# andrewdalpino/UltraZoom

Hardware: NVIDIA B200
Metric: output_mpx_per_s (higher is better)
Workload: dtype bf16

## Files before the change

### include/mewzoom_b200.h

```cpp
#ifndef MEWZOOM_B200_H_
#define MEWZOOM_B200_H_

#include <stddef.h>
#include <stdint.h>

#ifdef __cplusplus
extern "C" {
#endif

#define MZ_ABI_VERSION 4

typedef enum mz_status {
  MZ_OK = 0,
  MZ_ERR_INVALID = -1,
  MZ_ERR_CUDA = -2,
  MZ_ERR_UNSUPPORTED = -3,
  MZ_ERR_WORKSPACE = -4,
  MZ_ERR_STATE = -5
} mz_status;

#define MZ_FLAG_CLAMP01 1u
#define MZ_FLAG_SIMT_CONV 2u
#define MZ_FLAG_IO_U8 8u
#define MZ_FLAG_U8_TRUNC 16u
// ... 110 lines not shown
int mz_bicubic_f32(const float* x_dev, float* y_dev, int32_t planes, int32_t H, int32_t W, int32_t r,
                   void* stream);

int mz_stem_pack(const float* x_dev, const float* w_dev, const float* bias_dev, float* zf_dev, void* zb_dev,
                 int32_t B, int32_t H, int32_t W, int32_t Cp, int32_t zb_pitch, int32_t operand_dtype, void* stream);

int mz_conv3x3(const void* in_dev, const void* wpacked_dev, int32_t mode, const float* film_dev,
               void* out16_dev, float* zf_dev, int32_t B, int32_t H, int32_t W, int32_t cin_p, int32_t in_pitch,
               int32_t cout_p, int32_t out_pitch, int32_t zf_pitch, int32_t operand_dtype, int32_t use_tc,
               const mz_conv_tune* tune, void* stream);

int mz_head_shuffle_add(const void* zb_dev, const void* wpacked_dev, const float* x_dev, float* y_dev,
                        int32_t B, int32_t H, int32_t W, int32_t cin_p, int32_t in_pitch, int32_t r,
                        int32_t skip_mode, int32_t clamp01, int32_t operand_dtype, int32_t use_tc,
                        const mz_conv_tune* tune, void* stream);

int mz_yuv420_to_rgb16(const void* yuv_dev, uint16_t* rgb_dev, int32_t B, int32_t H, int32_t W, uint32_t flags, void* stream);
int mz_rgb16_to_yuv420(const uint16_t* rgb_dev, void* yuv_dev, int32_t B, int32_t H, int32_t W, uint32_t flags, void* stream);

int mz_pack_conv_weight(const float* w_host, int32_t cout, int32_t cin, int32_t cout_p, int32_t cin_p,
                        int32_t operand_dtype, void* dst_dev, size_t* bytes);

int mz_control_film(const float* c_dev, int32_t c_rows, const float* w_dev ,
                    const float* b_dev , float* film_dev , int32_t L, int32_t B,
                    int32_t F, int32_t hC, int32_t hCp, void* stream);

int mz_put_plane_async(void* dst, size_t dpitch, const void* src, size_t spitch, size_t width_bytes, size_t height,
                       void* stream);

int mz_ipc_frame_create(size_t bytes, void** dev_ptr, void* handle64);
int mz_ipc_frame_open(const void* handle64, void** dev_ptr);
int mz_ipc_frame_close(void* dev_ptr, int32_t owner);

#define MZ_MATH_TF32 0
#define MZ_MATH_FP32 1

int mz_adaptive_mix(const float* x_dev, const float* z_dev, const float* wt_dev, float alpha_logit, float* out_dev,
                    void* out16_dev, int64_t npix, int32_t C, int32_t pitch, int32_t operand_dtype, int32_t math, void* stream);

int mz_pixel_crush(const float* in_dev, const float* wt_dev, float* out_dev, void* out16_dev, int32_t B, int32_t H, int32_t W,
                   int32_t Cin, int32_t Cout, int32_t factor, int32_t pitch_in, int32_t pitch_out, int32_t operand_dtype,
                   int32_t math, void* stream);

int mz_quality_assessor(const float* in_dev, const float* wt_dev, const float* bias_dev, float* out_dev, int32_t B, int32_t H,
                        int32_t W, int32_t C, int32_t F, int32_t pitch_in, void* stream);

int mz_pixel_shuffle_nhwc(const float* in_dev, float* out_dev, void* out16_dev, int32_t B, int32_t H, int32_t W, int32_t C,
                          int32_t r, int32_t pitch_in, int32_t pitch_out, int32_t operand_dtype, void* stream);

int mz_crop_feature_maps(const float* in_dev, float* out_dev, int32_t B, int32_t H, int32_t W, int32_t C, int32_t target_h,
                         int32_t target_w, int32_t pitch_in, int32_t pitch_out, void* stream);

int mz_probe_umma(int32_t kc, int32_t row_shift, int32_t base_offset_mode, float* max_abs_err_out);
int mz_probe_set_gap(int32_t burst_iters, int32_t gap_cycles, int32_t commit_in_gap);
int mz_probe_mma_rate(int32_t n, int32_t kc, int32_t iters, int32_t ctas, int32_t distinct_a,
                      int32_t distinct_d, int32_t a_row_shift, float* cycles_per_mma_out);

int mz_padded_channels(int32_t c);

int mz_zb_pitch(int32_t cp);

#ifdef __cplusplus
}
#endif
#endif
```

### ultrazoom_b200/_native.py

```python
from __future__ import annotations

import ctypes as C
import os
import threading

_HERE = os.path.dirname(os.path.abspath(__file__))
LIB_PATH = os.path.join(_HERE, "lib", "libmewzoom_b200.so")

ABI_VERSION = 4

MZ_OK = 0
MZ_ERR_INVALID = -1
MZ_ERR_CUDA = -2
MZ_ERR_UNSUPPORTED = -3
MZ_ERR_WORKSPACE = -4
MZ_ERR_STATE = -5

FLAG_CLAMP01 = 1
FLAG_SIMT_CONV = 2
FLAG_SKIP_FROM_BUFFER = 4
FLAG_IO_U8 = 8
FLAG_U8_TRUNC = 16
FLAG_X_NHWC = 32
FLAG_Y_NHWC = 64
# ... 43 lines not shown
        ("fuse", C.c_int32),
        ("block", C.c_int32),
        ("seg_rows", C.c_int32),
    ]


_P = C.c_void_p
_I = C.c_int32
SIGNATURES = {
    "mz_last_error": (C.c_char_p, []),
    "mz_abi_version": (C.c_int, []),
    "mz_device_count": (C.c_int, []),
    "mz_model_create": (C.c_int, [C.POINTER(MzConfig), C.POINTER(_P)]),
    "mz_model_destroy": (None, [_P]),
    "mz_model_set_weight": (C.c_int, [_P, _I, _I, _P, C.c_size_t]),
    "mz_model_set_weight_dev": (C.c_int, [_P, _I, _I, _P, C.c_size_t, _P]),
    "mz_model_saturated": (C.c_int, [_P, _I, C.POINTER(_I)]),
    "mz_model_set_tune": (C.c_int, [_P, _I, C.POINTER(MzConvTune)]),
    "mz_model_enable_timing": (C.c_int, [_P, _I]),
    "mz_model_conv_stack_ms": (C.c_int, [_P, C.POINTER(C.c_float)]),
    "mz_workspace_bytes": (C.c_int, [_P, _I, _I, _I, C.POINTER(C.c_size_t)]),
    "mz_workspace_bytes_flags": (C.c_int, [_P, _I, _I, _I, C.c_uint32, C.POINTER(C.c_size_t)]),
    "mz_model_fused_block": (C.c_int, [_P]),
    "mz_block_fused": (C.c_int, [_P, _P, _P, _P, _P, _P, _I, _I, _I, _I, _I, _I, _P]),
    "mz_upscale": (C.c_int, [_P, _P, _P, _I, _P, _I, _I, _I, _P, C.c_size_t, C.c_uint32, _P]),
    "mz_upscale_window": (C.c_int, [_P, _P, _P, _I, _P, C.c_int64, C.c_int64, _I, _I, _I, _I, _I, _I, _I, _P, C.c_size_t,
                                    C.c_uint32, _P]),
    "mz_upscale_stage": (C.c_int, [_P, _P, _P, _I, _P, C.c_int64, C.c_int64, _I, _I, _I, _I, _I, _I, _I, _P, C.c_size_t,
                                   C.c_uint32, _P, _I, _I]),
    "mz_workspace_layout": (C.c_int, [_P, _I, _I, _I, C.POINTER(C.c_size_t), C.POINTER(C.c_size_t), C.POINTER(C.c_size_t),
                                      C.POINTER(_I), C.POINTER(_I)]),
    "mz_enable_peer_access": (C.c_int, [_I, _I]),
    "mz_ipc_frame_create": (C.c_int, [C.c_size_t, C.POINTER(C.c_void_p), _P]),
    "mz_ipc_frame_open": (C.c_int, [_P, C.POINTER(C.c_void_p)]),
    "mz_ipc_frame_close": (C.c_int, [_P, _I]),
    "mz_upscale_host": (C.c_int, [_P, _P, _P, _I, _P, _I, _I, _I, C.c_uint32]),
    "mz_upscale_host_async": (C.c_int, [_P, _I, _P, _P, _I, _P, _I, _I, _I, C.c_uint32]),
    "mz_upscale_host_wait": (C.c_int, [_P, _I]),
    "mz_put_plane_async": (C.c_int, [_P, C.c_size_t, _P, C.c_size_t, C.c_size_t, C.c_size_t, _P]),
    "mz_bicubic_f32": (C.c_int, [_P, _P, _I, _I, _I, _I, _P]),
    "mz_stem_pack": (C.c_int, [_P, _P, _P, _P, _P, _I, _I, _I, _I, _I, _I, _P]),
    "mz_conv3x3": (C.c_int, [_P, _P, _I, _P, _P, _P, _I, _I, _I, _I, _I, _I, _I, _I, _I, _I, C.POINTER(MzConvTune), _P]),
    "mz_head_shuffle_add": (C.c_int, [_P, _P, _P, _P, _I, _I, _I, _I, _I, _I, _I, _I, _I, _I, C.POINTER(MzConvTune), _P]),
    "mz_yuv420_to_rgb16": (C.c_int, [_P, _P, _I, _I, _I, C.c_uint32, _P]),
    "mz_rgb16_to_yuv420": (C.c_int, [_P, _P, _I, _I, _I, C.c_uint32, _P]),
    "mz_pack_conv_weight": (C.c_int, [_P, _I, _I, _I, _I, _I, _P, C.POINTER(C.c_size_t)]),
    "mz_control_film": (C.c_int, [_P, _I, _P, _P, _P, _I, _I, _I, _I, _I, _P]),
    "mz_adaptive_mix": (C.c_int, [_P, _P, _P, C.c_float, _P, _P, C.c_int64, _I, _I, _I, _I, _P]),
    "mz_pixel_crush": (C.c_int, [_P, _P, _P, _P, _I, _I, _I, _I, _I, _I, _I, _I, _I, _I, _P]),
    "mz_quality_assessor": (C.c_int, [_P, _P, _P, _P, _I, _I, _I, _I, _I, _I, _P]),
    "mz_pixel_shuffle_nhwc": (C.c_int, [_P, _P, _P, _I, _I, _I, _I, _I, _I, _I, _I, _P]),
    "mz_crop_feature_maps": (C.c_int, [_P, _P, _I, _I, _I, _I, _I, _I, _I, _I, _P]),
    "mz_probe_umma": (C.c_int, [_I, _I, _I, C.POINTER(C.c_float)]),
    "mz_probe_set_gap": (C.c_int, [_I, _I, _I]),
    "mz_probe_mma_rate": (C.c_int, [_I, _I, _I, _I, _I, _I, _I, C.POINTER(C.c_float)]),
    "mz_padded_channels": (C.c_int, [_I]),
    "mz_zb_pitch": (C.c_int, [_I]),
}

_lib = None
_lock = threading.Lock()


def load(build_if_missing: bool = True) -> C.CDLL:
    global _lib
    with _lock:
        if _lib is not None:
            return _lib
        if build_if_missing:
            from . import build as _build

            try:
                _build.build_locked()
            except RuntimeError:
                if not os.path.exists(LIB_PATH):
                    raise
        if not os.path.exists(LIB_PATH):
            raise RuntimeError(f"{LIB_PATH} is missing; run `python -m ultrazoom_b200.build`")
        try:
            lib = C.CDLL(LIB_PATH)
        except OSError as e:
            raise RuntimeError(f"cannot load {LIB_PATH}: {e}") from e
        for name, (res, args) in SIGNATURES.items():
            fn = getattr(lib, name)
            fn.restype = res
            fn.argtypes = args
        if lib.mz_abi_version() != ABI_VERSION:
            raise RuntimeError(f"ABI mismatch: library reports {lib.mz_abi_version()}, binding expects {ABI_VERSION}")
        _lib = lib
        return lib


def last_error() -> str:
    return load().mz_last_error().decode("utf-8", "replace")


def check(rc: int) -> None:
    if rc == MZ_OK:
        return
    msg = last_error()
    if rc == MZ_ERR_INVALID:
        raise AssertionError(msg)
    raise RuntimeError(f"mewzoom_b200 error {rc}: {msg}")


def dtype_code(dt) -> int:
# ... 14 lines not shown
```

### ultrazoom_b200/csrc/block_fused.cu

```cuda
#include <stdlib.h>

#include "kernels.cuh"

namespace mz {

namespace fb {
constexpr int kC = 48, kHC = 96;
constexpr int kStrip = 126;
constexpr int kThreads = 384;
constexpr int kZbStages = 4, kHidBufs = 2, kAcc1Stages = 2, kNB = 4, kRingBlocks = kNB + 2;
constexpr uint32_t kW1Tile = 48 * 32;
constexpr uint32_t kW1Bytes = 27 * kW1Tile;
constexpr uint32_t kW2Tile = 72 * 64;
constexpr uint32_t kW2Bytes = 9 * kW2Tile;
constexpr uint32_t kZbSub = 4352;
constexpr uint32_t kZbRow = 3 * kZbSub, kZbRowTx = 3 * 130 * 32;
constexpr uint32_t kHidChunk = 128 * 64, kHidBuf = 3 * kHidChunk;
constexpr uint32_t kStageZ = 3 * 32 * 64, kStageO = 3 * 32 * 32, kStageWarp = kStageZ + kStageO;

constexpr uint32_t oW1 = 0;
constexpr uint32_t oW2 = oW1 + kW1Bytes;
constexpr uint32_t oZb = oW2 + kW2Bytes;
constexpr uint32_t oHid = oZb + kZbStages * kZbRow;
constexpr uint32_t oStage = (oHid + kHidBufs * kHidBuf + 256 + 1023) & ~1023u;
// ... 171 lines not shown
          }
          if (leader) umma2_commit_mcast(bar_acc2_full + 8 * (pos % kNB), 3);
          __syncwarp();
        }
      }
      for (int i = 0; i <= steps; ++i) {
        if (i < steps) {
          for (int k = (i == 0 ? 0 : 2); k < 3; ++k) {
            const uint32_t c = zcnt + i + k;
            FB_TIMED(0, mbar_wait(bar_zb_full + 8 * (c % kZbStages), (c / kZbStages) & 1u));
          }
          const uint32_t st1 = a1 % kAcc1Stages;
          FB_TIMED(1, mbar_wait(bar_acc1_empty + 8 * st1, ((a1 / kAcc1Stages) & 1u) ^ 1u));
          tc_fence_after();
          const uint32_t d1 = tmem_base + kAcc1Col + st1 * kHC;
          if (leader) {
            if (!(p.dbg & 4))
#pragma unroll
            for (int dy = 0; dy < 3; ++dy) {
              const uint32_t arow = base + oZb + ((zcnt + i + dy) % kZbStages) * kZbRow;
#pragma unroll
              for (int dx = 0; dx < 3; ++dx) {
#pragma unroll
                for (int sub = 0; sub < 3; ++sub) {
                  const uint64_t ad = (static_cast<uint64_t>(hi32) << 32) | lo(arow + sub * kZbSub + dx * 32);
                  const uint64_t bd = (static_cast<uint64_t>(hi32) << 32) | lo(base + oW1 + ((dy * 3 + sub) * 3 + dx) * kW1Tile);
                  if (dy == 0 && dx == 0 && sub == 0)
                    umma2_bf16(d1, ad, bd, p.idesc1, 0u);
                  else
                    umma2_acc(d1, ad, bd, p.idesc1);
                }
              }
            }
            umma2_commit_mcast(bar_acc1_full + 8 * st1, 3);
            umma2_commit_mcast(bar_zb_empty + 8 * ((zcnt + i) % kZbStages), 3);
            if (i == steps - 1) {
              umma2_commit_mcast(bar_zb_empty + 8 * ((zcnt + i + 1) % kZbStages), 3);
              umma2_commit_mcast(bar_zb_empty + 8 * ((zcnt + i + 2) % kZbStages), 3);
            }
          }
          __syncwarp();
          ++a1;
        }
        if (i >= 1) {
          const int j = i - 1;
          const uint32_t hb = hcnt % kHidBufs;
          FB_TIMED(2, mbar_wait(bar_hid_full + 8 * hb, (hcnt / kHidBufs) & 1u));
          while (opened <= pos + j + 2) {
            FB_TIMED(3, mbar_wait(bar_acc2_empty + 8 * (opened % kNB), ((opened / kNB) & 1u) ^ 1u));
            ++opened;
          }
          tc_fence_after();
          const uint32_t d2 = tmem_base + kRingCol + ((pos + j) % kNB) * kC;
          if (leader) {
            if (!(p.dbg & 8))
#pragma unroll
            for (int dx = 0; dx < 3; ++dx) {
#pragma unroll
              for (int c = 0; c < 3; ++c) {
#pragma unroll
                for (int ks = 0; ks < 2; ++ks) {
                  const uint64_t ad = (static_cast<uint64_t>(hi64) << 32) | lo(base + oHid + hb * kHidBuf + c * kHidChunk + dx * 64 + ks * 32);
                  const uint64_t bd = (static_cast<uint64_t>(hi64) << 32) | lo(base + oW2 + (dx * 3 + c) * kW2Tile + ks * 32);
                  umma2_acc(d2, ad, bd, p.idesc2);
                }
              }
            }
            umma2_commit_mcast(bar_hid_empty + 8 * hb, 3);
            umma2_commit_mcast(bar_acc2_full + 8 * ((pos + j) % kNB), 3);
            if (j == steps - 1) {
              umma2_commit_mcast(bar_acc2_full + 8 * ((pos + j + 1) % kNB), 3);
              umma2_commit_mcast(bar_acc2_full + 8 * ((pos + j + 2) % kNB), 3);
            }
          }
          __syncwarp();
          ++hcnt;
        }
      }
      zcnt += rows_per_unit;
      pos += rows_per_unit;
    }
  } else if (warp >= 4 && warp < 8) {
    griddep_wait();
    const int q = warp & 3;
    float* film_s = reinterpret_cast<float*>(gen_base + oFilm);
    int film_b = -1;
    float amax = 0.f;
    uint32_t a1 = 0;
    const uint32_t px_row = q * 32 + lane;
    for (int unit = cluster_id; unit < p.n_units; unit += n_clusters) {
      int b, y0, x0;
      unit_geom(unit, b, y0, x0);
      if (b != film_b) {
        named_bar_sync(1, 128);
        for (int i = threadIdx.x - 128; i < 2 * kHC; i += 128) {
          float v = i < kHC ? 1.f : 0.f;
          if (p.film != nullptr) v = __ldg(p.film + static_cast<size_t>(b) * 2 * kHC + i);
          film_s[i] = 0.5f * v;
        }
        named_bar_sync(1, 128);
        film_b = b;
      }
      const int hx = x0 - 1 + static_cast<int>(px_row);
      const bool px_ok = hx >= 0 && hx < p.W;
      for (int i = 0; i < steps; ++i, ++a1) {
        const uint32_t st1 = a1 % kAcc1Stages, hb = a1 % kHidBufs;
        const int hy = y0 - 1 + i;
        const bool keep = px_ok && hy >= 0 && hy < p.H;
        FB_TIMED(0, mbar_wait(bar_acc1_full + 8 * st1, (a1 / kAcc1Stages) & 1u));
        FB_TIMED(1, mbar_wait(bar_hid_empty + 8 * hb, ((a1 / kHidBufs) & 1u) ^ 1u));
        __syncwarp();
        tc_fence_after();
        const uint32_t taddr = tmem_base + (static_cast<uint32_t>(q * 32) << 16) + kAcc1Col + st1 * kHC;
        const uint32_t hrow = base + oHid + hb * kHidBuf + px_row * 64;
#pragma unroll
        for (int c = 0; c < 3; ++c) {
          uint32_t v[32];
          FB_TIMED(2, { tmem_ld32(taddr + c * 32, v); tmem_ld_wait(); });
          const long long t_math = prof_on ? clock64() : 0;
          const float4* sc = reinterpret_cast<const float4*>(film_s + c * 32);
          const float4* sh = reinterpret_cast<const float4*>(film_s + kHC + c * 32);
          uint32_t o[16];
#pragma unroll
          for (int kk = 0; kk < 8; ++kk) {
            const float4 g = sc[kk], h = sh[kk];
            float a0 = silu_h(fmaf(__uint_as_float(v[4 * kk + 0]), g.x, h.x));
            float a1v = silu_h(fmaf(__uint_as_float(v[4 * kk + 1]), g.y, h.y));
            float a2 = silu_h(fmaf(__uint_as_float(v[4 * kk + 2]), g.z, h.z));
            float a3 = silu_h(fmaf(__uint_as_float(v[4 * kk + 3]), g.w, h.w));
            if (!keep) a0 = a1v = a2 = a3 = 0.f;
            if (p.dbg & 2) a0 = a1v = a2 = a3 = __uint_as_float(v[4 * kk]);
            amax = fmaxf(fmaxf(amax, fmaxf(fabsf(a0), fabsf(a1v))), fmaxf(fabsf(a2), fabsf(a3)));
            o[2 * kk] = pack_op2(p.bf16, a0, a1v);
            o[2 * kk + 1] = pack_op2(p.bf16, a2, a3);
          }
          const uint32_t crow = hrow + c * kHidChunk;
#pragma unroll
          for (int ch = 0; ch < 4; ++ch)
            sts128(crow + swz_chunk(px_row, ch, 64) * 16, o[4 * ch], o[4 * ch + 1], o[4 * ch + 2], o[4 * ch + 3]);
          if (prof_on) tick[3] += clock64() - t_math;
        }
        FB_TIMED(4, {
          tc_fence_before();
          fence_proxy_async_smem();
          __syncwarp();
        });
        FB_TIMED(5, {
          if (lane == 0) {
            mbar_arrive_remote(mapa_u32(bar_acc1_empty + 8 * st1, 0));
            mbar_arrive_remote(mapa_u32(bar_hid_full + 8 * hb, 0));
          }
        });
      }
    }
    if (!p.bf16 && p.sat != nullptr && !(amax <= MZ_F16_MAX)) *p.sat = 1u;
  } else if (warp >= 8) {
    griddep_wait();
    const int q = warp & 3;
    const uint32_t st_z = base + oStage + q * kStageWarp, st_o = st_z + kStageZ;
    const uint32_t my_res = bar_res + 8 * (q * 3);
    const CUtensorMap* tmZ = &p.tmZ[q == 3 ? 1 : 0];
    const CUtensorMap* tmO = &p.tmO[q == 3 ? 1 : 0];
    const uint32_t slice_bytes = (q == 3 ? 30u : 32u) * 16 * 4;
    float amax = 0.f;
    const bool lane_live = !(q == 3 && lane >= 30);
    uint32_t pos = 0, rpar = 0;
    bool preloaded = false;
    bool pending_last = false;
    for (int unit = cluster_id; unit < p.n_units; unit += n_clusters) {
      int b, y0, x0;
      unit_geom(unit, b, y0, x0);
      const int xw = x0 + q * 32;
      const int lead = static_cast<int>((static_cast<uint32_t>(y0 + 2) - pos) & 3u);
      for (int rho = -lead; rho < rows_per_unit; ++rho, ++pos) {
        const int y = y0 - 2 + rho;
        const bool store = rho >= 2 && rho < T + 2 && y < p.H && xw < p.W && !(p.dbg & 1);
        const uint32_t k = pos % kNB, par = (pos / kNB) & 1u;
        if (store && lane == 0) {
          if (!preloaded) {
            FB_TIMED(2, bulk_wait_read<0>());
            for (int j = 0; j < 3; ++j) {
              mbar_expect_tx(my_res + 8 * j, slice_bytes);
              tma_load_4d(st_z + j * 2048, tmZ, my_res + 8 * j, j * 16, xw, y, b);
            }
          } else if (pending_last) {
            FB_TIMED(2, bulk_wait_read<0>());
            mbar_expect_tx(my_res + 16, slice_bytes);
            tma_load_4d(st_z + 2 * 2048, tmZ, my_res + 16, 32, xw, y, b);
          }
        }
        FB_TIMED(0, mbar_wait(bar_acc2_full + 8 * k, par));
        __syncwarp();
        tc_fence_after();
        const long long t_body = prof_on ? clock64() : 0;
        const uint32_t lane_base = tmem_base + (static_cast<uint32_t>(q * 32) << 16) + kRingCol;
// ... 263 lines not shown
```

### ultrazoom_b200/csrc/common.cuh

```cuda
#pragma once

#include <cuda.h>
#include <cuda_bf16.h>
#include <cuda_fp16.h>
#include <cuda_runtime.h>
#include <stdint.h>
#include <stdio.h>

#include "../../include/mewzoom_b200.h"

namespace mz {

void set_error(const char* fmt, ...);
int cuda_fail(cudaError_t e, const char* what, const char* file, int line);

#define MZ_CUDA(expr)                                                        \
  do {                                                                       \
    cudaError_t _e = (expr);                                                 \
    if (_e != cudaSuccess) return ::mz::cuda_fail(_e, #expr, __FILE__, __LINE__); \
  } while (0)

#define MZ_REQUIRE(cond, ...)          \
  do {                                 \
    if (!(cond)) {                     \
// ... 170 lines not shown
__device__ __forceinline__ void mbar_arrive_cluster(uint32_t cluster_addr) {
  asm volatile("mbarrier.arrive.release.cluster.shared::cluster.b64 _, [%0];" ::"r"(cluster_addr) : "memory");
}
__device__ __forceinline__ void mbar_arrive_remote(uint32_t cluster_addr) {
  asm volatile("mbarrier.arrive.shared::cluster.b64 _, [%0];" ::"r"(cluster_addr) : "memory");
}
__device__ __forceinline__ void tma2_load_4d(uint32_t dst, const CUtensorMap* m, uint32_t bar_cluster, int c0, int c1,
                                             int c2, int c3) {
  asm volatile(
      "cp.async.bulk.tensor.4d.cta_group::2.shared::cluster.global.mbarrier::complete_tx::bytes [%0], [%1, {%3, %4, %5, "
      "%6}], [%2];" ::"r"(dst),
      "l"(reinterpret_cast<uint64_t>(m)), "r"(bar_cluster), "r"(c0), "r"(c1), "r"(c2), "r"(c3)
      : "memory");
}
__device__ __forceinline__ void tma2_load_3d(uint32_t dst, const CUtensorMap* m, uint32_t bar_cluster, int c0, int c1,
                                             int c2) {
  asm volatile(
      "cp.async.bulk.tensor.3d.cta_group::2.shared::cluster.global.mbarrier::complete_tx::bytes [%0], [%1, {%3, %4, "
      "%5}], [%2];" ::"r"(dst),
      "l"(reinterpret_cast<uint64_t>(m)), "r"(bar_cluster), "r"(c0), "r"(c1), "r"(c2)
      : "memory");
}
__device__ __forceinline__ void tmem_alloc2(uint32_t smem_dst, uint32_t ncols) {
  asm volatile("tcgen05.alloc.cta_group::2.sync.aligned.shared::cta.b32 [%0], %1;" ::"r"(smem_dst), "r"(ncols)
               : "memory");
}
__device__ __forceinline__ void tmem_relinquish2() {
  asm volatile("tcgen05.relinquish_alloc_permit.cta_group::2.sync.aligned;" ::: "memory");
}
__device__ __forceinline__ void tmem_dealloc2(uint32_t taddr, uint32_t ncols) {
  asm volatile("tcgen05.dealloc.cta_group::2.sync.aligned.b32 %0, %1;" ::"r"(taddr), "r"(ncols) : "memory");
}
__device__ __forceinline__ void umma2_bf16(uint32_t d_tmem, uint64_t a_desc, uint64_t b_desc, uint32_t idesc,
                                           uint32_t accumulate) {
  asm volatile(
      "{\n\t"
      ".reg .pred p;\n\t"
      "setp.ne.b32 p, %4, 0;\n\t"
      "tcgen05.mma.cta_group::2.kind::f16 [%0], %1, %2, %3, p;\n\t"
      "}\n" ::"r"(d_tmem),
      "l"(a_desc), "l"(b_desc), "r"(idesc), "r"(accumulate)
      : "memory");
}
__device__ __forceinline__ void umma2_acc(uint32_t d_tmem, uint64_t a_desc, uint64_t b_desc, uint32_t idesc) {
  asm volatile(
      "{\n\t"
      ".reg .pred p;\n\t"
      "setp.eq.u32 p, 0, 0;\n\t"
      "tcgen05.mma.cta_group::2.kind::f16 [%0], %1, %2, %3, p;\n\t"
      "}\n" ::"r"(d_tmem),
      "l"(a_desc), "l"(b_desc), "r"(idesc)
      : "memory");
}
__device__ __forceinline__ void umma2_commit_mcast(uint32_t bar, uint16_t cta_mask) {
  asm volatile(
      "tcgen05.commit.cta_group::2.mbarrier::arrive::one.shared::cluster.multicast::cluster.b64 [%0], %1;" ::"r"(bar),
      "h"(cta_mask)
      : "memory");
}

__device__ __forceinline__ void griddep_launch_dependents() { asm volatile("griddepcontrol.launch_dependents;" ::: "memory"); }
__device__ __forceinline__ void griddep_wait() { asm volatile("griddepcontrol.wait;" ::: "memory"); }

__device__ __forceinline__ void tmem_alloc(uint32_t smem_dst, uint32_t ncols) {
  asm volatile("tcgen05.alloc.cta_group::1.sync.aligned.shared::cta.b32 [%0], %1;" ::"r"(smem_dst), "r"(ncols)
               : "memory");
}
__device__ __forceinline__ void tmem_relinquish() {
  asm volatile("tcgen05.relinquish_alloc_permit.cta_group::1.sync.aligned;" ::: "memory");
}
__device__ __forceinline__ void tmem_dealloc(uint32_t taddr, uint32_t ncols) {
  asm volatile("tcgen05.dealloc.cta_group::1.sync.aligned.b32 %0, %1;" ::"r"(taddr), "r"(ncols) : "memory");
}
__device__ __forceinline__ void tc_fence_before() {
  asm volatile("tcgen05.fence::before_thread_sync;" ::: "memory");
}
__device__ __forceinline__ void tc_fence_after() {
  asm volatile("tcgen05.fence::after_thread_sync;" ::: "memory");
}
__device__ __forceinline__ void umma_bf16(uint32_t d_tmem, uint64_t a_desc, uint64_t b_desc, uint32_t idesc,
                                          uint32_t accumulate) {
  asm volatile(
      "{\n\t"
      ".reg .pred p;\n\t"
      "setp.ne.b32 p, %4, 0;\n\t"
      "tcgen05.mma.cta_group::1.kind::f16 [%0], %1, %2, %3, p;\n\t"
      "}\n" ::"r"(d_tmem),
      "l"(a_desc), "l"(b_desc), "r"(idesc), "r"(accumulate)
      : "memory");
}
__device__ __forceinline__ void umma_acc(uint32_t d_tmem, uint64_t a_desc, uint64_t b_desc, uint32_t idesc) {
  asm volatile(
      "{\n\t"
      ".reg .pred p;\n\t"
      "setp.eq.u32 p, 0, 0;\n\t"
      "tcgen05.mma.cta_group::1.kind::f16 [%0], %1, %2, %3, p;\n\t"
      "}\n" ::"r"(d_tmem),
      "l"(a_desc), "l"(b_desc), "r"(idesc)
      : "memory");
}
__device__ __forceinline__ void umma_commit(uint32_t bar) {
  asm volatile("tcgen05.commit.cta_group::1.mbarrier::arrive::one.shared::cluster.b64 [%0];" ::"r"(bar)
               : "memory");
}
__device__ __forceinline__ void umma_commit_mcast(uint32_t bar, uint16_t cta_mask) {
  asm volatile(
      "tcgen05.commit.cta_group::1.mbarrier::arrive::one.shared::cluster.multicast::cluster.b64 [%0], %1;" ::"r"(bar),
      "h"(cta_mask)
      : "memory");
}
__device__ __forceinline__ void tmem_ld16(uint32_t taddr, uint32_t (&v)[16]) {
  asm volatile(
      "tcgen05.ld.sync.aligned.32x32b.x16.b32 "
      "{%0, %1, %2, %3, %4, %5, %6, %7, %8, %9, %10, %11, %12, %13, %14, %15}, [%16];"
      : "=r"(v[0]), "=r"(v[1]), "=r"(v[2]), "=r"(v[3]), "=r"(v[4]), "=r"(v[5]), "=r"(v[6]), "=r"(v[7]),
        "=r"(v[8]), "=r"(v[9]), "=r"(v[10]), "=r"(v[11]), "=r"(v[12]), "=r"(v[13]), "=r"(v[14]), "=r"(v[15])
      : "r"(taddr)
      : "memory");
}
__device__ __forceinline__ void tmem_ld32(uint32_t taddr, uint32_t (&v)[32]) {
  asm volatile(
      "tcgen05.ld.sync.aligned.32x32b.x32.b32 "
      "{%0, %1, %2, %3, %4, %5, %6, %7, %8, %9, %10, %11, %12, %13, %14, %15, "
      "%16, %17, %18, %19, %20, %21, %22, %23, %24, %25, %26, %27, %28, %29, %30, %31}, [%32];"
      : "=r"(v[0]), "=r"(v[1]), "=r"(v[2]), "=r"(v[3]), "=r"(v[4]), "=r"(v[5]), "=r"(v[6]), "=r"(v[7]),
        "=r"(v[8]), "=r"(v[9]), "=r"(v[10]), "=r"(v[11]), "=r"(v[12]), "=r"(v[13]), "=r"(v[14]), "=r"(v[15]),
        "=r"(v[16]), "=r"(v[17]), "=r"(v[18]), "=r"(v[19]), "=r"(v[20]), "=r"(v[21]), "=r"(v[22]), "=r"(v[23]),
        "=r"(v[24]), "=r"(v[25]), "=r"(v[26]), "=r"(v[27]), "=r"(v[28]), "=r"(v[29]), "=r"(v[30]), "=r"(v[31])
      : "r"(taddr)
      : "memory");
}
__device__ __forceinline__ void tmem_ld_wait() {
  asm volatile("tcgen05.wait::ld.sync.aligned;" ::: "memory");
}
__device__ __forceinline__ void tmem_zero16(uint32_t taddr) {
  const uint32_t z = 0u;
  asm volatile(
      "tcgen05.st.sync.aligned.32x32b.x16.b32 [%0], "
      "{%1, %1, %1, %1, %1, %1, %1, %1, %1, %1, %1, %1, %1, %1, %1, %1};" ::"r"(taddr),
      "r"(z)
      : "memory");
}
__device__ __forceinline__ void tmem_st_wait() {
  asm volatile("tcgen05.wait::st.sync.aligned;" ::: "memory");
}

__host__ __device__ constexpr uint32_t umma_layout_type(int kc) { return kc == 64 ? 2u : (kc == 32 ? 4u : 6u); }

__device__ __forceinline__ uint64_t umma_smem_desc(uint32_t saddr, uint32_t sbo_bytes, uint32_t layout_type,
                                                   uint32_t base_offset = 0) {
  uint64_t d = 0;
  d |= static_cast<uint64_t>((saddr & 0x3FFFFu) >> 4);
  d |= static_cast<uint64_t>(1) << 16;
  d |= static_cast<uint64_t>((sbo_bytes >> 4) & 0x3FFFu) << 32;
  d |= static_cast<uint64_t>(1) << 46;
  d |= static_cast<uint64_t>(base_offset & 7u) << 49;
  d |= static_cast<uint64_t>(layout_type & 7u) << 61;
  return d;
}
__host__ __device__ constexpr uint32_t umma_idesc_bf16(int m, int n) {
  return (1u << 4) | (1u << 7) | (1u << 10) | (static_cast<uint32_t>(n >> 3) << 17) |
         (static_cast<uint32_t>(m >> 4) << 24);
}
__host__ __device__ constexpr uint32_t umma_idesc_f16(int m, int n) {
  return (1u << 4) | (static_cast<uint32_t>(n >> 3) << 17) | (static_cast<uint32_t>(m >> 4) << 24);
}

__device__ __forceinline__ uint32_t pack_bf16x2(float lo, float hi) {
  __nv_bfloat162 v = __floats2bfloat162_rn(lo, hi);
  return *reinterpret_cast<uint32_t*>(&v);
}
__device__ __forceinline__ uint32_t pack_f16x2(float lo, float hi) {
  uint32_t r;
  asm("cvt.rn.satfinite.f16x2.f32 %0, %1, %2;" : "=r"(r) : "f"(hi), "f"(lo));
  return r;
}
__device__ __forceinline__ uint32_t pack_f16x2_rn(float lo, float hi) {
  uint32_t r;
  asm("cvt.rn.f16x2.f32 %0, %1, %2;" : "=r"(r) : "f"(hi), "f"(lo));
  return r;
}
__device__ __forceinline__ uint32_t pack_op2(int bf16, float lo, float hi) {
  return bf16 ? pack_bf16x2(lo, hi) : pack_f16x2(lo, hi);
}
__device__ __forceinline__ uint32_t pack_shadow2(int bf16, float lo, float hi) {
  return bf16 ? pack_bf16x2(lo, hi) : pack_f16x2_rn(lo, hi);
}
__device__ __forceinline__ float2 unpack_op2(int bf16, uint32_t u) {
  if (bf16) return make_float2(__uint_as_float(u << 16), __uint_as_float(u & 0xffff0000u));
  return __half22float2(*reinterpret_cast<const __half2*>(&u));
}
__device__ __forceinline__ float op_to_float(int bf16, uint16_t v) {
  return bf16 ? __uint_as_float(static_cast<uint32_t>(v) << 16) : __half2float(__ushort_as_half(v));
// ... 22 lines not shown
```

### ultrazoom_b200/csrc/probe.cu

```cuda
#include <vector>

#include "kernels.cuh"

namespace mz {

constexpr int kProbeRows = 384;
constexpr int kProbeN = 64;

struct ProbeParams {
  CUtensorMap tmA, tmB;
  float* out;
  int kc, row_shift, bo_mode;
};

__global__ void __launch_bounds__(128, 1) probe_umma_kernel(const __grid_constant__ ProbeParams p) {
  extern __shared__ uint8_t smem_raw[];
  const uint32_t raw = smem_u32(smem_raw);
  const uint32_t base = (raw + 1023u) & ~1023u;
  uint8_t* gen = smem_raw + (base - raw);
  const int row_bytes = p.kc * 2;
  const uint32_t a_smem = base;
  const uint32_t b_smem = base + kProbeRows * 128;
  const uint32_t bar_full = b_smem + kProbeN * 128;
  const uint32_t bar_done = bar_full + 8;
  const uint32_t tmem_slot = bar_done + 32;
  volatile uint32_t* tmem_gen = reinterpret_cast<volatile uint32_t*>(gen + (tmem_slot - base));
  const int warp = threadIdx.x >> 5, lane = threadIdx.x & 31;

  if (threadIdx.x == 0) {
    mbar_init(bar_full, 1);
    mbar_init(bar_done, 1);
    fence_mbar_init();
  }
  if (warp == 0) {
    tmem_alloc(tmem_slot, 64);
    tmem_relinquish();
  }
  tc_fence_before();
  __syncthreads();
  tc_fence_after();
  const uint32_t tmem_base = *tmem_gen;

  if (threadIdx.x == 0) {
    mbar_expect_tx(bar_full, (kProbeRows + kProbeN) * row_bytes);
    tma_load_2d(a_smem, &p.tmA, bar_full, 0, 0);
    tma_load_2d(a_smem + 192 * row_bytes, &p.tmA, bar_full, 0, 192);
    tma_load_2d(b_smem, &p.tmB, bar_full, 0, 0);
    mbar_wait(bar_full, 0);
    tc_fence_after();
    const uint32_t lt = umma_layout_type(p.kc);
    const uint32_t sbo = 8u * row_bytes;
    const uint32_t idesc = umma_idesc_bf16(128, kProbeN);
    for (int ks = 0; ks < p.kc / 16; ++ks) {
      const uint32_t a_addr = a_smem + p.row_shift * row_bytes + ks * 32;
      const uint32_t bo = p.bo_mode ? ((a_addr >> 7) & 7u) : 0u;
      umma_bf16(tmem_base, umma_smem_desc(a_addr, sbo, lt, bo), umma_smem_desc(b_smem + ks * 32, sbo, lt, 0), idesc,
                ks != 0);
    }
    umma_commit(bar_done);
  }
  mbar_wait(bar_done, 0);
  __syncwarp();
  tc_fence_after();
  const uint32_t taddr = tmem_base + (static_cast<uint32_t>(warp * 32) << 16);
  for (int n0 = 0; n0 < kProbeN; n0 += 16) {
    uint32_t v[16];
    tmem_ld16(taddr + n0, v);
    tmem_ld_wait();
#pragma unroll
    for (int i = 0; i < 16; ++i) p.out[(warp * 32 + lane) * kProbeN + n0 + i] = __uint_as_float(v[i]);
  }
  tc_fence_before();
  __syncthreads();
  if (warp == 0) {
    tc_fence_after();
    tmem_dealloc(tmem_base, 64);
  }
}

struct RateParams {
  float* out;
  int n, kc, iters, distinct_a, distinct_d, a_row_shift;
  int gap_cycles, commit_in_gap;
  int burst_iters;
  uint32_t tmem_cols;
};

__global__ void __launch_bounds__(128, 1) probe_rate_kernel(const RateParams p) {
  extern __shared__ uint8_t smem_raw[];
  const uint32_t raw = smem_u32(smem_raw);
  const uint32_t base = (raw + 1023u) & ~1023u;
  uint8_t* gen = smem_raw + (base - raw);
  const uint32_t a_smem = base;
  const uint32_t b_smem = base + 8 * 16384;
  const uint32_t bar_done = b_smem + 32768;
  const uint32_t tmem_slot = bar_done + 32;
  volatile uint32_t* tmem_gen = reinterpret_cast<volatile uint32_t*>(gen + (tmem_slot - base));
  const int warp = threadIdx.x >> 5;
  for (uint32_t i = threadIdx.x; i < (8 * 16384 + 32768) / 4; i += blockDim.x)
    reinterpret_cast<uint32_t*>(gen)[i] = 0x3c003c00u;
  fence_proxy_async_smem();
  if (threadIdx.x == 0) {
    mbar_init(bar_done, 1);
    mbar_init(bar_done + 16, 1);
    fence_mbar_init();
  }
  if (warp == 0) {
    tmem_alloc(tmem_slot, p.tmem_cols);
    tmem_relinquish();
  }
  tc_fence_before();
  __syncthreads();
  tc_fence_after();
  const uint32_t tmem_base = *tmem_gen;
  if (warp == 1) {
    const int row_bytes = p.kc * 2;
    const uint32_t lt = umma_layout_type(p.kc);
    const uint32_t sbo = 8u * row_bytes;
    const uint32_t idesc = umma_idesc_bf16(128, p.n);
    const uint32_t hi = static_cast<uint32_t>(umma_smem_desc(0, sbo, lt, 0) >> 32);
    const uint32_t lo0 = static_cast<uint32_t>(umma_smem_desc(0, sbo, lt, 0));
    const uint32_t b_lo = lo0 + (b_smem >> 4);
    const uint32_t a_lo = lo0 + ((a_smem + static_cast<uint32_t>(p.a_row_shift * row_bytes)) >> 4);
    const uint32_t a_step = p.distinct_a > 1 ? (16384u >> 4) : 0u;
    const uint32_t d_step = p.distinct_d > 1 ? static_cast<uint32_t>(p.n) : 0u;
    const bool leader = elect_one();
    const uint32_t dynmask = (p.iters & 1) ? 0xffffffffu : static_cast<uint32_t>(p.a_row_shift >> 8);
    const long long t0 = clock64();
    int until_gap = p.burst_iters;
// ... 52 lines not shown
    hB[i] = __float2bfloat16_rn(fB[i]);
  }
  __nv_bfloat16 *dA = nullptr, *dB = nullptr;
  float* dOut = nullptr;
  MZ_CUDA(cudaMalloc(&dA, hA.size() * 2));
  MZ_CUDA(cudaMalloc(&dB, hB.size() * 2));
  MZ_CUDA(cudaMalloc(&dOut, sizeof(float) * 128 * kProbeN));
  MZ_CUDA(cudaMemcpy(dA, hA.data(), hA.size() * 2, cudaMemcpyHostToDevice));
  MZ_CUDA(cudaMemcpy(dB, hB.data(), hB.size() * 2, cudaMemcpyHostToDevice));
  MZ_CUDA(cudaMemset(dOut, 0xff, sizeof(float) * 128 * kProbeN));
  ProbeParams p;
  memset(&p, 0, sizeof(p));
  p.out = dOut;
  p.kc = kc;
  p.row_shift = row_shift;
  p.bo_mode = base_offset_mode;
  const CUtensorMapSwizzle swz =
      kc == 64 ? CU_TENSOR_MAP_SWIZZLE_128B : (kc == 32 ? CU_TENSOR_MAP_SWIZZLE_64B : CU_TENSOR_MAP_SWIZZLE_32B);
  int rc;
  {
    const uint64_t dims[2] = {static_cast<uint64_t>(kc), kProbeRows};
    const uint64_t strides[1] = {static_cast<uint64_t>(kc) * 2};
    const uint32_t box[2] = {static_cast<uint32_t>(kc), 192};
    rc = encode_tmap(&p.tmA, CU_TENSOR_MAP_DATA_TYPE_BFLOAT16, 2, dA, dims, strides, box, swz);
  }
  if (rc == MZ_OK) {
    const uint64_t dims[2] = {static_cast<uint64_t>(kc), kProbeN};
    const uint64_t strides[1] = {static_cast<uint64_t>(kc) * 2};
    const uint32_t box[2] = {static_cast<uint32_t>(kc), kProbeN};
    rc = encode_tmap(&p.tmB, CU_TENSOR_MAP_DATA_TYPE_BFLOAT16, 2, dB, dims, strides, box, swz);
  }
  if (rc == MZ_OK) {
    const int smem = 1024 + kProbeRows * 128 + kProbeN * 128 + 64;
    cudaError_t e = cudaFuncSetAttribute(probe_umma_kernel, cudaFuncAttributeMaxDynamicSharedMemorySize, smem);
    if (e == cudaSuccess) {
      probe_umma_kernel<<<1, 128, smem>>>(p);
      e = cudaGetLastError();
    }
    if (e == cudaSuccess) e = cudaDeviceSynchronize();
    if (e != cudaSuccess) rc = cuda_fail(e, "probe_umma_kernel", __FILE__, __LINE__);
  }
  if (rc == MZ_OK) {
    std::vector<float> out(128 * kProbeN);
    cudaMemcpy(out.data(), dOut, out.size() * sizeof(float), cudaMemcpyDeviceToHost);
    float worst = 0.f;
    for (int m = 0; m < 128; ++m)
      for (int n = 0; n < kProbeN; ++n) {
        float ref = 0.f;
        for (int k = 0; k < kc; ++k) ref += fA[static_cast<size_t>(row_shift + m) * kc + k] * fB[static_cast<size_t>(n) * kc + k];
        float d = fabsf(out[m * kProbeN + n] - ref);
        if (!(d == d)) d = 1e30f;
        if (d > worst) worst = d;
      }
    *max_abs_err_out = worst;
  }
  cudaFree(dA);
  cudaFree(dB);
  cudaFree(dOut);
  return rc;
}

static int g_gap_cycles = 0, g_commit_in_gap = 0, g_burst_iters = 0;
int mz_probe_set_gap(int32_t burst_iters, int32_t gap_cycles, int32_t commit_in_gap) {
  g_burst_iters = burst_iters;
  g_gap_cycles = gap_cycles;
  g_commit_in_gap = commit_in_gap;
  return MZ_OK;
}

int mz_probe_mma_rate(int32_t n, int32_t kc, int32_t iters, int32_t ctas, int32_t distinct_a, int32_t distinct_d,
                      int32_t a_row_shift, float* cycles_per_mma_out) {
  MZ_REQUIRE(a_row_shift >= 0 && a_row_shift <= 64, "probe: a_row_shift must be in [0, 64]");
  MZ_REQUIRE(n >= 16 && n <= 256 && n % 16 == 0, "probe: n must be a multiple of 16 in [16, 256]");
  MZ_REQUIRE(kc == 16 || kc == 32 || kc == 64, "probe: kc must be 16, 32 or 64");
  MZ_REQUIRE(iters > 0 && iters <= (1 << 20) && ctas > 0 && ctas <= 4096, "probe: bad iters/ctas");
  MZ_REQUIRE(distinct_a == 1 || distinct_a == 2 || distinct_a == 4 || distinct_a == 8, "probe: distinct_a must be 1, 2, 4 or 8");
  MZ_REQUIRE(distinct_d >= 1 && distinct_d * n <= 512, "probe: distinct_d * n must fit 512 TMEM columns");
  MZ_REQUIRE(cycles_per_mma_out, "probe: null output");
  float* dOut = nullptr;
  MZ_CUDA(cudaMalloc(&dOut, sizeof(float) * ctas));
  RateParams p;
  p.out = dOut;
  p.n = n;
  p.kc = kc;
  p.iters = iters;
  p.distinct_a = distinct_a;
  p.distinct_d = distinct_d;
  p.a_row_shift = a_row_shift;
  p.gap_cycles = g_gap_cycles;
  p.commit_in_gap = g_commit_in_gap;
  p.burst_iters = g_burst_iters;
  p.tmem_cols = 32;
  while (p.tmem_cols < static_cast<uint32_t>(n * distinct_d)) p.tmem_cols <<= 1;
  const int smem = 1024 + 8 * 16384 + 32768 + 128;
  int rc = MZ_OK;
  cudaError_t e = cudaFuncSetAttribute(probe_rate_kernel, cudaFuncAttributeMaxDynamicSharedMemorySize, smem);
  if (e == cudaSuccess) {
    probe_rate_kernel<<<ctas, 128, smem>>>(p);
    e = cudaGetLastError();
  }
  if (e == cudaSuccess) e = cudaDeviceSynchronize();
  if (e != cudaSuccess) rc = cuda_fail(e, "probe_rate_kernel", __FILE__, __LINE__);
  if (rc == MZ_OK) {
    std::vector<float> out(ctas);
    cudaMemcpy(out.data(), dOut, sizeof(float) * ctas, cudaMemcpyDeviceToHost);
    double sum = 0;
// ... 9 lines not shown
```

### ultrazoom_b200/ops.py

```python
from __future__ import annotations

import ctypes as C
from typing import Optional

import torch
from torch import Tensor

from . import _native


def _stream(t: Tensor) -> int:
    return torch.cuda.current_stream(t.device).cuda_stream


def _need_cuda(*ts: Tensor) -> None:
    for t in ts:
        if t is not None and not t.is_cuda:
            raise RuntimeError("ultrazoom_b200.ops: CUDA tensors required (no CPU fallback)")


def padded_channels(c: int) -> int:
    return _native.load().mz_padded_channels(c)


# ... 117 lines not shown
            inp.data_ptr(), wpacked.data_ptr(), mode, film.data_ptr() if film is not None else None,
            out.data_ptr() + 2 * channel_offset, zf.data_ptr() + 4 * channel_offset if zf is not None else None, B, H, W, cin_p,
            in_pitch if in_pitch != cin_p else 0, cout_p, out_pitch if out_pitch != cout_p else 0,
            zf_pitch if zf_pitch != cout_p else 0, _native.dtype_code(inp.dtype), 1 if use_tc else 0,
            C.byref(tune) if tune is not None else None, _stream(inp)))
    return out


def block_fused(zb: Tensor, w1_packed: Tensor, w2_packed: Tensor, film: Optional[Tensor], zf: Tensor, seg_rows: int = 0,
                max_ctas: int = 0) -> Tensor:
    _need_cuda(zb, w1_packed, w2_packed, zf)
    assert zb.dtype in (torch.float16, torch.bfloat16) and w1_packed.dtype == zb.dtype and w2_packed.dtype == zb.dtype
    zb = zb.contiguous()
    B, H, W, Cc = zb.shape
    assert Cc == 48 and tuple(w1_packed.shape) == (9, 96, 48) and tuple(w2_packed.shape) == (9, 48, 96), "48 / 96 channels only"
    assert zf.is_contiguous() and tuple(zf.shape) == (B, H, W, 48) and zf.dtype == torch.float32
    out = torch.empty_like(zb)
    with torch.cuda.device(zb.device):
        _native.check(_native.load().mz_block_fused(
            zb.data_ptr(), out.data_ptr(), zf.data_ptr(), w1_packed.data_ptr(), w2_packed.data_ptr(),
            film.data_ptr() if film is not None else None, B, H, W, _native.dtype_code(zb.dtype), seg_rows, max_ctas,
            _stream(zb)))
    return out


def head_shuffle_add(zb: Tensor, wpacked: Tensor, r: int, x: Optional[Tensor] = None, y: Optional[Tensor] = None,
                     skip_mode: int = 2, clamp01: bool = False, use_tc: bool = True,
                     tune: Optional[_native.MzConvTune] = None) -> Tensor:
    _need_cuda(zb, wpacked)
    assert zb.dtype in (torch.float16, torch.bfloat16) and wpacked.dtype == zb.dtype
    zb = zb.contiguous()
    B, H, W, in_pitch = zb.shape
    cin_p = wpacked.shape[2]
    assert in_pitch >= cin_p, "weight / activation channel mismatch"
    if y is None:
        assert skip_mode != 1, "skip_mode 1 needs y preloaded with the bicubic image"
        y = torch.empty((B, 3, H * r, W * r), dtype=torch.float32, device=zb.device)
    if x is not None:
        x = x.to(torch.float32).contiguous()
    with torch.cuda.device(zb.device):
        _native.check(_native.load().mz_head_shuffle_add(
            zb.data_ptr(), wpacked.data_ptr(), x.data_ptr() if x is not None else None, y.data_ptr(), B, H, W, cin_p,
            in_pitch if in_pitch != cin_p else 0, r, skip_mode, 1 if clamp01 else 0, _native.dtype_code(zb.dtype), 1 if use_tc else 0, C.byref(tune) if tune is not None else None,
            _stream(zb)))
    return y


def probe_umma(kc: int, row_shift: int, base_offset_mode: int) -> float:
    err = C.c_float()
    _native.check(_native.load().mz_probe_umma(kc, row_shift, base_offset_mode, C.byref(err)))
    return err.value


def probe_mma_rate(n: int, kc: int, iters: int = 2000, ctas: int = 1, distinct_a: int = 1,
                   distinct_d: int = 1, a_row_shift: int = 0) -> float:
    cyc = C.c_float()
    _native.check(_native.load().mz_probe_mma_rate(n, kc, iters, ctas, distinct_a, distinct_d, a_row_shift,
                                                   C.byref(cyc)))
    return cyc.value
```

Baseline: 1108.

## Feed center-tap A operand of fused block second conv from TMEM

In the fused block kernel, the epilogue now also writes the activated hidden tile into TMEM alongside the swizzled shared-memory copy. For the dx==0 taps, the second conv's MMA reads its A operand from TMEM instead of a shared-memory descriptor, which is meant to cut shared-memory read bandwidth pressure on the tensor core. A probe kernel is added to check that TMEM-sourced A produces the same results as SMEM A. The cost is extra tcgen05.st traffic and a store wait in the epilogue. It also risks correctness, since the TMEM A layout and the ring-slot lifetime may not match what the MMA expects.

```diff
diff --git a/include/mewzoom_b200.h b/include/mewzoom_b200.h
--- a/include/mewzoom_b200.h
+++ b/include/mewzoom_b200.h
@@ -186,6 +186,7 @@
                          int32_t target_w, int32_t pitch_in, int32_t pitch_out, void* stream);
 
 int mz_probe_umma(int32_t kc, int32_t row_shift, int32_t base_offset_mode, float* max_abs_err_out);
+int mz_probe_umma_tmem_a(int32_t n, int32_t bf16, int32_t a_col, int32_t* mismatches_out, float* max_abs_err_out);
 int mz_probe_set_gap(int32_t burst_iters, int32_t gap_cycles, int32_t commit_in_gap);
 int mz_probe_mma_rate(int32_t n, int32_t kc, int32_t iters, int32_t ctas, int32_t distinct_a,
                       int32_t distinct_d, int32_t a_row_shift, float* cycles_per_mma_out);
diff --git a/ultrazoom_b200/_native.py b/ultrazoom_b200/_native.py
--- a/ultrazoom_b200/_native.py
+++ b/ultrazoom_b200/_native.py
@@ -119,6 +119,7 @@
     "mz_pixel_shuffle_nhwc": (C.c_int, [_P, _P, _P, _I, _I, _I, _I, _I, _I, _I, _I, _P]),
     "mz_crop_feature_maps": (C.c_int, [_P, _P, _I, _I, _I, _I, _I, _I, _I, _I, _P]),
     "mz_probe_umma": (C.c_int, [_I, _I, _I, C.POINTER(C.c_float)]),
+    "mz_probe_umma_tmem_a": (C.c_int, [_I, _I, _I, C.POINTER(C.c_int32), C.POINTER(C.c_float)]),
     "mz_probe_set_gap": (C.c_int, [_I, _I, _I]),
     "mz_probe_mma_rate": (C.c_int, [_I, _I, _I, _I, _I, _I, _I, C.POINTER(C.c_float)]),
     "mz_padded_channels": (C.c_int, [_I]),
diff --git a/ultrazoom_b200/csrc/block_fused.cu b/ultrazoom_b200/csrc/block_fused.cu
--- a/ultrazoom_b200/csrc/block_fused.cu
+++ b/ultrazoom_b200/csrc/block_fused.cu
@@ -247,6 +247,7 @@
           }
           tc_fence_after();
           const uint32_t d2 = tmem_base + kRingCol + ((pos + j) % kNB) * kC;
+          const uint32_t hid_t = tmem_base + kAcc1Col + (hcnt % kAcc1Stages) * kHC;
           if (leader) {
             if (!(p.dbg & 8))
 #pragma unroll
@@ -255,9 +256,13 @@
               for (int c = 0; c < 3; ++c) {
 #pragma unroll
                 for (int ks = 0; ks < 2; ++ks) {
-                  const uint64_t ad = (static_cast<uint64_t>(hi64) << 32) | lo(base + oHid + hb * kHidBuf + c * kHidChunk + dx * 64 + ks * 32);
                   const uint64_t bd = (static_cast<uint64_t>(hi64) << 32) | lo(base + oW2 + (dx * 3 + c) * kW2Tile + ks * 32);
-                  umma2_acc(d2, ad, bd, p.idesc2);
+                  if (dx == 0) {
+                    umma2_tmem_a_acc(d2, hid_t + (2 * c + ks) * 8, bd, p.idesc2);
+                  } else {
+                    const uint64_t ad = (static_cast<uint64_t>(hi64) << 32) | lo(base + oHid + hb * kHidBuf + c * kHidChunk + dx * 64 + ks * 32);
+                    umma2_acc(d2, ad, bd, p.idesc2);
+                  }
                 }
               }
             }
@@ -333,9 +338,11 @@
 #pragma unroll
           for (int ch = 0; ch < 4; ++ch)
             sts128(crow + swz_chunk(px_row, ch, 64) * 16, o[4 * ch], o[4 * ch + 1], o[4 * ch + 2], o[4 * ch + 3]);
+          tmem_st16(taddr + 16 * c, o);
           if (prof_on) tick[3] += clock64() - t_math;
         }
         FB_TIMED(4, {
+          tmem_st_wait();
           tc_fence_before();
           fence_proxy_async_smem();
           __syncwarp();
diff --git a/ultrazoom_b200/csrc/common.cuh b/ultrazoom_b200/csrc/common.cuh
--- a/ultrazoom_b200/csrc/common.cuh
+++ b/ultrazoom_b200/csrc/common.cuh
@@ -246,6 +246,27 @@
       "l"(a_desc), "l"(b_desc), "r"(idesc)
       : "memory");
 }
+__device__ __forceinline__ void umma2_tmem_a(uint32_t d_tmem, uint32_t a_tmem, uint64_t b_desc, uint32_t idesc,
+                                             uint32_t accumulate) {
+  asm volatile(
+      "{\n\t"
+      ".reg .pred p;\n\t"
+      "setp.ne.b32 p, %4, 0;\n\t"
+      "tcgen05.mma.cta_group::2.kind::f16 [%0], [%1], %2, %3, p;\n\t"
+      "}\n" ::"r"(d_tmem),
+      "r"(a_tmem), "l"(b_desc), "r"(idesc), "r"(accumulate)
+      : "memory");
+}
+__device__ __forceinline__ void umma2_tmem_a_acc(uint32_t d_tmem, uint32_t a_tmem, uint64_t b_desc, uint32_t idesc) {
+  asm volatile(
+      "{\n\t"
+      ".reg .pred p;\n\t"
+      "setp.eq.u32 p, 0, 0;\n\t"
+      "tcgen05.mma.cta_group::2.kind::f16 [%0], [%1], %2, %3, p;\n\t"
+      "}\n" ::"r"(d_tmem),
+      "r"(a_tmem), "l"(b_desc), "r"(idesc)
+      : "memory");
+}
 __device__ __forceinline__ void umma2_commit_mcast(uint32_t bar, uint16_t cta_mask) {
   asm volatile(
       "tcgen05.commit.cta_group::2.mbarrier::arrive::one.shared::cluster.multicast::cluster.b64 [%0], %1;" ::"r"(bar),
@@ -333,6 +354,14 @@
       "tcgen05.st.sync.aligned.32x32b.x16.b32 [%0], "
       "{%1, %1, %1, %1, %1, %1, %1, %1, %1, %1, %1, %1, %1, %1, %1, %1};" ::"r"(taddr),
       "r"(z)
+      : "memory");
+}
+__device__ __forceinline__ void tmem_st16(uint32_t taddr, const uint32_t (&v)[16]) {
+  asm volatile(
+      "tcgen05.st.sync.aligned.32x32b.x16.b32 [%0], "
+      "{%1, %2, %3, %4, %5, %6, %7, %8, %9, %10, %11, %12, %13, %14, %15, %16};" ::"r"(taddr),
+      "r"(v[0]), "r"(v[1]), "r"(v[2]), "r"(v[3]), "r"(v[4]), "r"(v[5]), "r"(v[6]), "r"(v[7]), "r"(v[8]), "r"(v[9]),
+      "r"(v[10]), "r"(v[11]), "r"(v[12]), "r"(v[13]), "r"(v[14]), "r"(v[15])
       : "memory");
 }
 __device__ __forceinline__ void tmem_st_wait() {
diff --git a/ultrazoom_b200/csrc/probe.cu b/ultrazoom_b200/csrc/probe.cu
--- a/ultrazoom_b200/csrc/probe.cu
+++ b/ultrazoom_b200/csrc/probe.cu
@@ -75,6 +75,102 @@
   if (warp == 0) {
     tc_fence_after();
     tmem_dealloc(tmem_base, 64);
+  }
+}
+
+constexpr uint32_t kTaD1 = 0, kTaCol = 144, kTaD2 = 256;
+struct TmemAParams {
+  const uint16_t* a;
+  const uint16_t* b;
+  float* out;
+  int n, bf16, a_col;
+};
+
+__global__ void __cluster_dims__(2, 1, 1) __launch_bounds__(128, 1) probe_tmem_a_kernel(const __grid_constant__ TmemAParams p) {
+  __shared__ __align__(1024) uint8_t a_s[128 * 64];
+  __shared__ __align__(1024) uint8_t b_s[128 * 64];
+  __shared__ __align__(8) uint64_t bar[1];
+  __shared__ uint32_t tmem_slot;
+  const int warp = threadIdx.x >> 5, lane = threadIdx.x & 31;
+  const uint32_t rank = cluster_ctarank();
+  const int row = warp * 32 + lane;
+  const int nh = p.n / 2;
+  {
+    const uint4* src = reinterpret_cast<const uint4*>(p.a + (static_cast<size_t>(rank) * 128 + row) * 32);
+    for (int ch = 0; ch < 4; ++ch) {
+      const uint4 v = src[ch];
+      sts128(smem_u32(a_s) + row * 64 + swz_chunk(row, ch, 64) * 16, v.x, v.y, v.z, v.w);
+    }
+    if (row < nh) {
+      const uint4* bs = reinterpret_cast<const uint4*>(p.b + (static_cast<size_t>(rank) * nh + row) * 32);
+      for (int ch = 0; ch < 4; ++ch) {
+        const uint4 v = bs[ch];
+        sts128(smem_u32(b_s) + row * 64 + swz_chunk(row, ch, 64) * 16, v.x, v.y, v.z, v.w);
+      }
+    }
+  }
+  if (threadIdx.x == 0) {
+    mbar_init(smem_u32(bar), 1);
+    fence_mbar_init();
+  }
+  if (warp == 0) {
+    tmem_alloc2(smem_u32(&tmem_slot), 512);
+    tmem_relinquish2();
+  }
+  tc_fence_before();
+  __syncthreads();
+  tc_fence_after();
+  const uint32_t tmem_base = tmem_slot;
+  const uint32_t lane_addr = tmem_base + (static_cast<uint32_t>(warp * 32) << 16);
+  {
+    const uint32_t* src = reinterpret_cast<const uint32_t*>(p.a + (static_cast<size_t>(rank) * 128 + row) * 32);
+    uint32_t v[16];
+#pragma unroll
+    for (int w = 0; w < 16; ++w) v[w] = src[w];
+    tmem_st16(lane_addr + kTaCol + p.a_col, v);
+    tmem_st_wait();
+  }
+  fence_proxy_async_smem();
+  tc_fence_before();
+  cluster_sync_all();
+  tc_fence_after();
+  if (rank == 0 && warp == 0) {
+    if (elect_one()) {
+      const uint32_t idesc = p.bf16 ? umma_idesc_bf16(256, p.n) : umma_idesc_f16(256, p.n);
+      const uint64_t hi = umma_smem_desc(0, 8 * 64, umma_layout_type(32), 0) & 0xFFFFFFFF00000000ull;
+      const uint64_t lo0 = umma_smem_desc(0, 8 * 64, umma_layout_type(32), 0) & 0x3FFF0000ull;
+      for (int ks = 0; ks < 2; ++ks) {
+        const uint64_t ad = hi | lo0 | ((smem_u32(a_s) + ks * 32) & 0x3FFFFu) >> 4;
+        const uint64_t bd = hi | lo0 | ((smem_u32(b_s) + ks * 32) & 0x3FFFFu) >> 4;
+        umma2_bf16(tmem_base + kTaD1, ad, bd, idesc, ks != 0);
+      }
+      for (int ks = 0; ks < 2; ++ks) {
+        const uint64_t bd = hi | lo0 | ((smem_u32(b_s) + ks * 32) & 0x3FFFFu) >> 4;
+        umma2_tmem_a(tmem_base + kTaD2, tmem_base + kTaCol + p.a_col + 8 * ks, bd, idesc, ks != 0);
+      }
+      umma2_commit_mcast(smem_u32(bar), 3);
+    }
+    __syncwarp();
+  }
+  mbar_wait(smem_u32(bar), 0);
+  __syncwarp();
+  tc_fence_after();
+  for (int path = 0; path < 2; ++path) {
+    float* dst = p.out + (static_cast<size_t>(path) * 256 + rank * 128 + row) * p.n;
+    for (int n0 = 0; n0 < p.n; n0 += 16) {
+      uint32_t v[16];
+      tmem_ld16(lane_addr + (path ? kTaD2 : kTaD1) + n0, v);
+      tmem_ld_wait();
+#pragma unroll
+      for (int i = 0; i < 16; ++i) dst[n0 + i] = __uint_as_float(v[i]);
+    }
+  }
+  tc_fence_before();
+  __syncthreads();
+  cluster_sync_all();
+  if (warp == 0) {
+    tc_fence_after();
+    tmem_dealloc2(tmem_base, 512);
   }
 }
 
@@ -233,6 +329,75 @@
         if (!(d == d)) d = 1e30f;
         if (d > worst) worst = d;
       }
+    *max_abs_err_out = worst;
+  }
+  cudaFree(dA);
+  cudaFree(dB);
+  cudaFree(dOut);
+  return rc;
+}
+
+int mz_probe_umma_tmem_a(int32_t n, int32_t bf16, int32_t a_col, int32_t* mismatches_out, float* max_abs_err_out) {
+  MZ_REQUIRE(n >= 32 && n <= static_cast<int>(kTaCol) && n % 16 == 0, "probe: n must be a multiple of 16 in [32, 144]");
+  MZ_REQUIRE(a_col >= 0 && a_col % 8 == 0 && kTaCol + a_col + 16 <= kTaD2, "probe: a_col must be a multiple of 8 in [0, 96]");
+  MZ_REQUIRE(mismatches_out && max_abs_err_out, "probe: null output");
+  std::vector<uint16_t> hA(256 * 32), hB(static_cast<size_t>(n) * 32);
+  std::vector<float> fA(hA.size()), fB(hB.size());
+  uint32_t s = 24680u;
+  auto fill = [&](std::vector<uint16_t>& h, std::vector<float>& f) {
+    for (size_t i = 0; i < h.size(); ++i) {
+      s = s * 1664525u + 1013904223u;
+      f[i] = static_cast<float>(static_cast<int>((s >> 16) % 257) - 128) / 64.f;
+      if (bf16) {
+        const __nv_bfloat16 v = __float2bfloat16_rn(f[i]);
+        h[i] = *reinterpret_cast<const uint16_t*>(&v);
+      } else {
+        const __half v = __float2half_rn(f[i]);
+        h[i] = *reinterpret_cast<const uint16_t*>(&v);
+      }
+    }
+  };
+  fill(hA, fA);
+  fill(hB, fB);
+  uint16_t *dA = nullptr, *dB = nullptr;
+  float* dOut = nullptr;
+  const size_t n_out = 2 * 256 * static_cast<size_t>(n);
+  MZ_CUDA(cudaMalloc(&dA, hA.size() * 2));
+  MZ_CUDA(cudaMalloc(&dB, hB.size() * 2));
+  MZ_CUDA(cudaMalloc(&dOut, sizeof(float) * n_out));
+  MZ_CUDA(cudaMemcpy(dA, hA.data(), hA.size() * 2, cudaMemcpyHostToDevice));
+  MZ_CUDA(cudaMemcpy(dB, hB.data(), hB.size() * 2, cudaMemcpyHostToDevice));
+  MZ_CUDA(cudaMemset(dOut, 0xff, sizeof(float) * n_out));
+  TmemAParams p;
+  p.a = dA;
+  p.b = dB;
+  p.out = dOut;
+  p.n = n;
+  p.bf16 = bf16 ? 1 : 0;
+  p.a_col = a_col;
+  int rc = MZ_OK;
+  probe_tmem_a_kernel<<<2, 128>>>(p);
+  cudaError_t e = cudaGetLastError();
+  if (e == cudaSuccess) e = cudaDeviceSynchronize();
+  if (e != cudaSuccess) rc = cuda_fail(e, "probe_tmem_a_kernel", __FILE__, __LINE__);
+  if (rc == MZ_OK) {
+    std::vector<float> out(n_out);
+    cudaMemcpy(out.data(), dOut, out.size() * sizeof(float), cudaMemcpyDeviceToHost);
+    int mism = 0;
+    float worst = 0.f;
+    for (int m = 0; m < 256; ++m)
+      for (int j = 0; j < n; ++j) {
+        const float x = out[static_cast<size_t>(m) * n + j], y = out[(256 + static_cast<size_t>(m)) * n + j];
+        if (__builtin_memcmp(&x, &y, sizeof(float)) != 0) ++mism;
+        float ref = 0.f;
+        for (int k = 0; k < 32; ++k) ref += fA[static_cast<size_t>(m) * 32 + k] * fB[static_cast<size_t>(j) * 32 + k];
+        for (float v : {x, y}) {
+          float d = fabsf(v - ref);
+          if (!(d == d)) d = 1e30f;
+          if (d > worst) worst = d;
+        }
+      }
+    *mismatches_out = mism;
     *max_abs_err_out = worst;
   }
   cudaFree(dA);
diff --git a/ultrazoom_b200/ops.py b/ultrazoom_b200/ops.py
--- a/ultrazoom_b200/ops.py
+++ b/ultrazoom_b200/ops.py
@@ -193,6 +193,12 @@
     return err.value
 
 
+def probe_umma_tmem_a(n: int, bf16: bool, a_col: int = 0) -> tuple[int, float]:
+    mism, err = C.c_int32(), C.c_float()
+    _native.check(_native.load().mz_probe_umma_tmem_a(n, 1 if bf16 else 0, a_col, C.byref(mism), C.byref(err)))
+    return mism.value, err.value
+
+
 def probe_mma_rate(n: int, kc: int, iters: int = 2000, ctas: int = 1, distinct_a: int = 1,
                    distinct_d: int = 1, a_row_shift: int = 0) -> float:
     cyc = C.c_float()
```

After: 1115 (median of 6 runs). No clear change (+0.6%).
